# DeepGraphLearning/ultra_torchdrug

Hardware: AMD Instinct MI355X
Metric: edges aggregated/sec, FB15k237-shaped 6L x 64d rspmm Bellman-Ford (predict: the reference's 18 rspmm layers per batch as 6 relation-graph + 6 entity-graph launches, tails and heads in one pass) (higher is better)
Workload: dtype f32

## Files before the change

ultra_torchdrug_amd/csrc/plan_path.h:

```cpp
#ifndef ULTRA_PLAN_PATH_H
#define ULTRA_PLAN_PATH_H

#include <cstddef>
#include <cstdint>

#include "ultra_rspmm.h"

namespace ultra_detail {

constexpr int kTile = 64;
constexpr int kXcd = 8;
constexpr int kMaxLdsBytes = 156 * 1024;
constexpr int kLdsHeader = 16;
constexpr int kPlanBlock = 1024;
constexpr int kPlanRgBlock = 512;

enum Kind { KIND_FWD = 0, KIND_DX = 1, KIND_DREL = 2 };
enum Family { FAM_DENSE = 0, FAM_ROWGROUP = 1, FAM_QUAD = 2, FAM_PACKED = 3, FAM_GENERAL = 4 };
enum RelMode { REL_L2 = 0, REL_LDS = 1, REL_PART = 2 };
enum ActMode { ACT_NONE = 0, ACT_BITS = 2, ACT_NODE = 3 };
enum UnrollClass { UNROLL_U = 0, UNROLL_UW = 1, UNROLL_UX = 2 };
enum Fixup { FIX_NONE = 0, FIX_PLAIN = 1, FIX_MANY = 2 };

struct Knobs {
    bool force_general = false;
    bool no_x_lds = false;
    bool no_quad = false;
    bool no_rowgroup = false;
    bool wide_groups = false;
    bool no_concurrent_tiles = false;
    bool no_dense = false;
    bool no_dead_words = false;
};

inline Knobs decode_knobs(int mask) {
    Knobs k;
    k.force_general = (mask & 1) != 0;
    k.no_x_lds = (mask & 2) != 0;
    k.no_quad = (mask & 4) != 0;
    k.no_rowgroup = (mask & 8) != 0;
    k.wide_groups = (mask & 16) != 0;
    k.no_concurrent_tiles = (mask & 32) != 0;
    k.no_dense = (mask & 64) != 0;
    k.no_dead_words = (mask & 128) != 0;
    return k;
}

inline int gcd_int(int a, int b) {
    while (b) {
        const int t = a % b;
        a = b;
        b = t;
    }
    return a;
}

struct TileGeometry {
    int n_tiles = 0, split = 0, n_slots = 0, blocks_per_label = 0, grid = 0;
};

inline TileGeometry tile_geometry(long long columns, int width, int n_cu) {
    TileGeometry g;
    g.n_tiles = (int)((columns + width - 1) / width);
    g.split = kXcd / gcd_int(g.n_tiles, kXcd);
    g.n_slots = g.n_tiles * g.split;
    g.blocks_per_label = (n_cu + kXcd - 1) / kXcd;
    g.grid = g.blocks_per_label * kXcd;
    return g;
}

struct RowGroupTiling {
    int group = 16;
    int rel_mode = REL_L2;
    int n_rel_lds = 0;
    TileGeometry geo;
    size_t lds = 0;
};

inline RowGroupTiling rowgroup_tiling(long long F, long long gather_rows, long long n_rows, long long n_rel, int n_cu,
                                      bool wide_groups, size_t lds_base, size_t lds_room) {
    RowGroupTiling t;
    const bool dram = wide_groups || (double)gather_rows * (double)F * 4.0 > 256.0 * 1024 * 1024;
    t.group = (dram && F % 256 == 0) ? 64 : ((dram && F % 128 == 0) ? 32 : 16);
    const int width = 4 * t.group;
    t.geo = tile_geometry(F, width, n_cu);
    while ((n_rows + t.geo.split - 1) / t.geo.split * F * 4 >= (1LL << 32) - 65536 && t.geo.split < (1 << 20)) t.geo.split *= 2;
    t.geo.n_slots = t.geo.n_tiles * t.geo.split;
    const size_t row_bytes = (size_t)width * sizeof(float);
    const size_t lds_need = (size_t)n_rel * row_bytes;
    const int part_rows = (int)(lds_room / row_bytes);
    t.lds = lds_base;
    if (n_rel > 0 && lds_need <= lds_room) {
        t.rel_mode = REL_LDS;
        t.n_rel_lds = (int)n_rel;
        t.lds += lds_need;
    } else if (n_rel > 0 && (long long)part_rows * 4 >= n_rel) {
        t.rel_mode = REL_PART;
        t.n_rel_lds = part_rows;
        t.lds += (size_t)part_rows * row_bytes;
    }
    return t;
}

enum Aligned {
    AL_INPUT = 1, AL_GRAD = 2, AL_OUT = 4, AL_RELATION = 8, AL_ADD_ROWS = 16, AL_PARTIAL = 32, AL_BVEC = 64, AL_ALL = 127
};

struct PlanInput {
    int kind = KIND_FWD, sum_op = ULTRA_SUM_ADD, mul_op = ULTRA_MUL_MUL;
    long long F = 0, n_rel = 0, gather_rows = 0, gather2_rows = 0;
    bool has_weight = false, has_node_b = false, has_row_ptr = false, has_packed = false, has_packed_dead = false,
         has_dense = false;
    long long packed_src_shift = 0, n_rows = 0, n_edges = 0, n_long_rows = 0, n_pieces = 0, n_hot = 0, dense_rows = 0,
              dense_cols = 0;
    bool has_add_rows = false, has_bnode = false;
    int bdim = 0;
    bool has_act_bits = false, has_act_node = false;
    int act_words = 0;
    bool has_workspace = false;
    size_t workspace_bytes = 0;
    unsigned aligned = AL_ALL;
    Knobs knobs;
    int n_cu = 0;
    bool gfx950 = false;
};

struct PlanPath {
    int status = ULTRA_OK;
    int family = FAM_GENERAL;
    bool unit_w = false;
    int var = 0;
    bool x_lds = false, dead = false;
    int act = ACT_NONE;
    int unroll = UNROLL_U;
    int concurrent = 1;
    bool rel_lds = false;
    int group = 0, rel_mode = REL_L2, n_rel_lds = 0;
    TileGeometry geo;
    int grid = 0, block = 0;
    size_t lds = 0;
    int fixup = FIX_NONE, fixup_grid = 0;
};

inline void set_rowgroup(PlanPath &r, const RowGroupTiling &t) {
    r.family = FAM_ROWGROUP;
    r.group = t.group; r.rel_mode = t.rel_mode; r.n_rel_lds = t.n_rel_lds;
    r.geo = t.geo; r.grid = t.geo.grid; r.block = kPlanRgBlock; r.lds = t.lds;
}

inline bool dense_applies(const PlanInput &c) {
    if (!c.has_dense || c.has_weight || c.sum_op != ULTRA_SUM_ADD || c.n_rel != 4) return false;
    if (c.F % 16 != 0 || c.F * 4 >= (1LL << 24)) return false;
    if (c.dense_cols != c.gather_rows || c.gather_rows * c.F * 4 >= (1LL << 31)) return false;
    if (c.kind == KIND_DREL) {
        if (c.mul_op != ULTRA_MUL_MUL || c.n_rows != 4 || c.dense_rows != c.gather2_rows) return false;
        const long long n_vt = (c.dense_rows + 15) / 16;
        if (!c.has_workspace || c.workspace_bytes < (size_t)(n_vt * 4 * c.F) * sizeof(float)) return false;
    } else {
        if (c.dense_rows != c.n_rows) return false;
        if (c.kind == KIND_FWD && !c.has_add_rows && c.has_bnode && c.bdim <= 0) return false;
    }
    return true;
}

inline void force_concurrent(PlanPath &path, int want, bool has_min_rows, long long min_rows, long long gather_rows) {
    if (path.family == FAM_QUAD && want >= 1 && path.geo.blocks_per_label % want == 0 && (!has_min_rows || gather_rows >= min_rows))
        path.concurrent = want;
}

inline PlanPath plan_path(const PlanInput &in) {
    PlanPath r;
    const int kind = in.kind;
    const long long F = in.F, n_rel = in.n_rel;
    const Knobs &k = in.knobs;
    auto aligned = [&](unsigned bits) { return (in.aligned & bits) == bits; };
    const unsigned al_gather = (kind == KIND_DX) ? AL_GRAD : AL_INPUT;
    const bool sum_add = in.sum_op == ULTRA_SUM_ADD, mul_mul = in.mul_op == ULTRA_MUL_MUL;
    const bool boundary_ok = !in.has_bnode || in.bdim % 4 == 0;

    r.geo = tile_geometry(F, kTile, in.n_cu);
    r.grid = r.geo.grid;
    r.block = kPlanBlock;
    r.unit_w = !in.has_weight;
    const size_t lds_need = (size_t)n_rel * kTile * sizeof(float);
    const bool rel_fits = n_rel > 0 && lds_need <= (size_t)kMaxLdsBytes;

    if (in.has_dense && !k.no_dense && !k.force_general && !k.no_quad && !k.no_x_lds && in.gfx950 && dense_applies(in)) {
        r.family = FAM_DENSE;
        return r;
    }

    const bool big = in.packed_src_shift >= 32;
    if (kind != KIND_DREL && !k.force_general && !k.no_rowgroup && in.has_row_ptr && big && in.n_long_rows == 0 && F % 4 == 0 &&
        (kind == KIND_FWD || sum_add) && aligned(al_gather | AL_OUT | AL_RELATION | AL_ADD_ROWS | AL_BVEC) && boundary_ok) {
        r.family = FAM_ROWGROUP;
        if (F >= (1LL << 30)) { r.status = ULTRA_ERR_BAD_SHAPE; return r; }
        const bool needs_rel = kind == KIND_FWD || mul_mul;
// ... 81 lines not shown
```

ultra_torchdrug_amd/csrc/rspmm_kernels.hip:

```cpp
#include <hip/hip_runtime.h>
#include <type_traits>

#include <algorithm>
#include <cstdint>
#include <cstdlib>
#include <cstring>
#include <mutex>

#include "host_common.h"
#include "launch_record.h"

thread_local int ultra_detail_last_hip_error = 0;

namespace {

using namespace ultra_detail;

#ifndef ULTRA_BLOCK
#define ULTRA_BLOCK 1024
#endif
constexpr int kBlock = ULTRA_BLOCK;
#ifndef ULTRA_UNROLL
#define ULTRA_UNROLL 8
#endif
// ... 648 lines not shown
        }
#pragma unroll
        for (int q = 0; q < 8; ++q) {
            const int r = 4 * q + (lane >> 4), c = (lane & 15) * 4;
            long long gr = t * kCbRows + r;
            gr = gr < last ? gr : last;
            if constexpr (BND == 0) {
                pa[q] = *reinterpret_cast<const f32x4 *>(p.input + gr * 64 + c);
            } else {
                const unsigned qq = (unsigned)(query0 + r);
                const unsigned step = p.rpn >= kCbRows ? (qq >= (unsigned)p.rpn ? 1u : 0u) : qq / (unsigned)p.rpn;
                const int query = (int)(qq - step * (unsigned)p.rpn);
                const f32x4 zero = {0.0f, 0.0f, 0.0f, 0.0f};
                if constexpr (BND == 1) {
                    const f32x4 v = *reinterpret_cast<const f32x4 *>(bv_lds + query * 64 + c);
                    pa[q] = (node0 + step == (long long)bn_lds[query]) ? v : zero;
                } else {
                    pa[q] = (node0 + step == (long long)p.in_bnode[query]) ? *reinterpret_cast<const f32x4 *>(p.in_bvec + query * 64 + c) : zero;
                }
            }
            pb[q] = *reinterpret_cast<const f32x4 *>(p.update + gr * 64 + c);
        }
    };
    if constexpr (PF) {
        if (wave_global < n_tiles) fetch(wave_global);
    }
    for (long long t = wave_global; t < n_tiles; t += wave_total) {
        const long long row0 = t * kCbRows;
        if constexpr (!PF) fetch(t);
#pragma unroll
        for (int q = 0; q < 8; ++q) {
            const int r = 4 * q + (lane >> 4), c = (lane & 15) * 4;
            *reinterpret_cast<f32x4 *>(tile + r * kCbStride + c) = pa[q];
            *reinterpret_cast<f32x4 *>(tile + r * kCbStride + 64 + c) = pb[q];
        }
        if constexpr (PF) {
            asm volatile("s_waitcnt lgkmcnt(0)" ::: "memory");
            if (t + wave_total < n_tiles) fetch(t + wave_total);
        } else {
            asm volatile("s_waitcnt vmcnt(0) lgkmcnt(0)" ::: "memory");
        }

        f32x16 acc0, acc1;
#pragma unroll
        for (int r = 0; r < 16; ++r) { acc0[r] = bias0; acc1[r] = bias1; }
#pragma unroll
        for (int q = 0; q < 16; ++q) {
            const f32x4 av = *reinterpret_cast<const f32x4 *>(tile + i * kCbStride + 64 * h + 4 * q);
            acc0 = __builtin_amdgcn_mfma_f32_32x32x2f32(av.x, w0[4 * q + 0], acc0, 0, 0, 0);
            acc1 = __builtin_amdgcn_mfma_f32_32x32x2f32(av.x, w1[4 * q + 0], acc1, 0, 0, 0);
            acc0 = __builtin_amdgcn_mfma_f32_32x32x2f32(av.y, w0[4 * q + 1], acc0, 0, 0, 0);
            acc1 = __builtin_amdgcn_mfma_f32_32x32x2f32(av.y, w1[4 * q + 1], acc1, 0, 0, 0);
            acc0 = __builtin_amdgcn_mfma_f32_32x32x2f32(av.z, w0[4 * q + 2], acc0, 0, 0, 0);
            acc1 = __builtin_amdgcn_mfma_f32_32x32x2f32(av.z, w1[4 * q + 2], acc1, 0, 0, 0);
            acc0 = __builtin_amdgcn_mfma_f32_32x32x2f32(av.w, w0[4 * q + 3], acc0, 0, 0, 0);
            acc1 = __builtin_amdgcn_mfma_f32_32x32x2f32(av.w, w1[4 * q + 3], acc1, 0, 0, 0);
        }
        asm volatile("s_waitcnt lgkmcnt(0)" ::: "memory");

#pragma unroll
        for (int r = 0; r < 16; ++r) {
            const int row = (r & 3) + 8 * (r >> 2) + 4 * h;
            tile[row * kCbStride + 64 + i] = acc0[r];
            tile[row * kCbStride + 96 + i] = acc1[r];
        }
        asm volatile("s_waitcnt lgkmcnt(0)" ::: "memory");

        float v[32];
#pragma unroll
        for (int q = 0; q < 8; ++q) {
            const f32x4 d = *reinterpret_cast<const f32x4 *>(tile + ln_row * kCbStride + 64 + 32 * ln_half + 4 * q);
            v[4 * q + 0] = d.x; v[4 * q + 1] = d.y; v[4 * q + 2] = d.z; v[4 * q + 3] = d.w;
            if constexpr (ZOUT) {
                const long long left_z = p.rows - row0;
                const __amdgpu_buffer_rsrc_t rsrc_z = __builtin_amdgcn_make_buffer_rsrc(
                    p.z_out + row0 * 64, 0, (int)(left_z < kCbRows ? left_z : kCbRows) * 256, 0x00020000);
                __builtin_amdgcn_raw_buffer_store_b128(__builtin_bit_cast(qu4, d), rsrc_z, ln_row * 256 + ln_half * 128 + 16 * q, 0, 0);
            }
        }
        if (p.gamma != nullptr) {
            float s = 0.0f;
#pragma unroll
            for (int c = 0; c < 32; ++c) s = s + v[c];
            const float so = __shfl_xor(s, 1, 64);
            const float mean = (ln_half == 0 ? s + so : so + s) * (1.0f / 64.0f);
            float ss = 0.0f;
#pragma unroll
            for (int c = 0; c < 32; ++c) { const float dlt = v[c] - mean; ss = ss + dlt * dlt; }
            const float sso = __shfl_xor(ss, 1, 64);
            const float var = (ln_half == 0 ? ss + sso : sso + ss) * (1.0f / 64.0f);
            const float inv = 1.0f / sqrtf(var + p.eps);
#pragma unroll
            for (int q = 0; q < 8; ++q) {
                const f32x4 gq = *reinterpret_cast<const f32x4 *>(gb + 32 * ln_half + 4 * q);
                const f32x4 bq = *reinterpret_cast<const f32x4 *>(gb + 64 + 32 * ln_half + 4 * q);
                v[4 * q + 0] = ((v[4 * q + 0] - mean) * inv) * gq.x + bq.x;
                v[4 * q + 1] = ((v[4 * q + 1] - mean) * inv) * gq.y + bq.y;
                v[4 * q + 2] = ((v[4 * q + 2] - mean) * inv) * gq.z + bq.z;
                v[4 * q + 3] = ((v[4 * q + 3] - mean) * inv) * gq.w + bq.w;
            }
        }
        if (p.relu) {
#pragma unroll
            for (int c = 0; c < 32; ++c) v[c] = !(v[c] <= 0.0f) ? v[c] : 0.0f;
        }
        if (p.shortcut) {
#pragma unroll
            for (int q = 0; q < 8; ++q) {
                const f32x4 x = *reinterpret_cast<const f32x4 *>(tile + ln_row * kCbStride + 32 * ln_half + 4 * q);
                v[4 * q + 0] = v[4 * q + 0] + x.x; v[4 * q + 1] = v[4 * q + 1] + x.y;
                v[4 * q + 2] = v[4 * q + 2] + x.z; v[4 * q + 3] = v[4 * q + 3] + x.w;
            }
        }
#pragma unroll
        for (int q = 0; q < 8; ++q) {
            f32x4 d;
            d.x = v[4 * q + 0]; d.y = v[4 * q + 1]; d.z = v[4 * q + 2]; d.w = v[4 * q + 3];
            *reinterpret_cast<f32x4 *>(tile + ln_row * kCbStride + 64 + 32 * ln_half + 4 * q) = d;
        }
        asm volatile("s_waitcnt lgkmcnt(0)" ::: "memory");

        if constexpr (BND == 3) {
            if (p.rows * 256 >= (1LL << 32) - 65536) {
#pragma unroll
                for (int q = 0; q < 8; ++q) {
                    const int r = 4 * q + (lane >> 4), c = (lane & 15) * 4;
                    const f32x4 d = *reinterpret_cast<const f32x4 *>(tile + r * kCbStride + 64 + c);
                    if (rid[q] >= 0) *reinterpret_cast<f32x4 *>(p.out + (long long)rid[q] * 64 + c) = d;
                }
                asm volatile("s_waitcnt lgkmcnt(0)" ::: "memory");
                continue;
            }
            const __amdgpu_buffer_rsrc_t rsrc_all = __builtin_amdgcn_make_buffer_rsrc(p.out, 0, (int)(uint32_t)(p.rows * 256), 0x00020000);
#pragma unroll
            for (int q = 0; q < 8; ++q) {
                const int r = 4 * q + (lane >> 4), c = (lane & 15) * 4;
                const f32x4 d = *reinterpret_cast<const f32x4 *>(tile + r * kCbStride + 64 + c);
                const uint32_t off = rid[q] >= 0 ? (uint32_t)rid[q] * 256u + (uint32_t)c * 4u : 0xffffffffu;
                __builtin_amdgcn_raw_buffer_store_b128(__builtin_bit_cast(qu4, d), rsrc_all, off, 0, 0);
            }
            asm volatile("s_waitcnt lgkmcnt(0)" ::: "memory");
            continue;
        }
        const long long left = p.rows - row0;
        const __amdgpu_buffer_rsrc_t rsrc_tile = __builtin_amdgcn_make_buffer_rsrc(
            p.out + row0 * 64, 0, (int)(left < kCbRows ? left : kCbRows) * 256, 0x00020000);
#pragma unroll
        for (int q = 0; q < 8; ++q) {
            const int r = 4 * q + (lane >> 4), c = (lane & 15) * 4;
            const f32x4 d = *reinterpret_cast<const f32x4 *>(tile + r * kCbStride + 64 + c);
            __builtin_amdgcn_raw_buffer_store_b128(__builtin_bit_cast(qu4, d), rsrc_tile, r * 256 + c * 4, 0, 0);
        }
        asm volatile("s_waitcnt lgkmcnt(0)" ::: "memory");
    }
}


static_assert(kBlock == kPlanBlock && kRgBlock == kPlanRgBlock, "plan_path.h states the workgroup sizes of its families");
static_assert(kRelL2 == REL_L2 && kRelLds == REL_LDS && kRelPart == REL_PART, "plan_path.h's RelMode is rowgroup.inc's REL");

thread_local hipEvent_t g_prof_start = nullptr;
thread_local hipEvent_t g_prof_stop = nullptr;
#ifndef ULTRA_QUAD_U
#define ULTRA_QUAD_U 8
#endif
constexpr int kQuadU = ULTRA_QUAD_U;
#ifndef ULTRA_QUAD_UW
#define ULTRA_QUAD_UW 6
#endif
constexpr int kQuadUW = ULTRA_QUAD_UW;
#ifndef ULTRA_QUAD_UX
#define ULTRA_QUAD_UX 8
#endif
constexpr int kQuadUX = ULTRA_QUAD_UX;

thread_local LaunchRing g_launches;

template <typename Kern, typename Params>
int launch_recorded(LaunchRecord rec, Kern kern, const Params &p, int grid, size_t lds, hipStream_t stream, int block) {
    rec.grid = grid; rec.block = block; rec.lds = (int32_t)lds;
    rec.n_tiles = p.n_tiles; rec.split = p.split; rec.n_slots = p.n_slots; rec.blocks_per_label = p.blocks_per_label;
    LaunchRecord &slot = g_launches.push(rec);
    return slot.status = launch_with_lds(kern, p, grid, lds, stream, block);
}


template <int KIND, int SUM, int MUL>
int launch_general(const KParams &p, const PlanPath &path, hipStream_t stream) {
    return with_bool(path.unit_w, [&](auto uw) {
        return with_bool(path.rel_lds, [&](auto rl) {
            constexpr bool UW = decltype(uw)::value, RL = decltype(rl)::value;
            if constexpr (RL && (KIND == KIND_DREL || (KIND == KIND_DX && SUM == ULTRA_SUM_ADD && MUL == ULTRA_MUL_ADD)))
                return (int)ULTRA_ERR_BAD_OP;
            else {
                LaunchRecord rec;
                rec.family = FAM_GENERAL; rec.kind = KIND; rec.sum = SUM; rec.mul = MUL; rec.unit_w = UW; rec.rel_lds = RL;
                return launch_recorded(rec, segment_kernel<KIND, SUM, MUL, UW, RL>, p, path.grid, path.lds, stream, kBlock);
            }
        });
    });
}

template <int KIND, int SUM, int MUL>
int launch_packed(const PParams &p, const PlanPath &path, hipStream_t stream) {
    return with_bool(path.unit_w, [&](auto uw) {
        auto go = [&](auto var) {
            constexpr int V = decltype(var)::value;
            constexpr int UN = (V == 2 || V == 3) ? kUnrollBig : kUnroll;
            constexpr bool UW = decltype(uw)::value;
            if constexpr (KIND == KIND_DX && MUL == ULTRA_MUL_ADD && V == 2) return (int)ULTRA_ERR_BAD_OP;
            else {
                LaunchRecord rec;
                rec.family = FAM_PACKED; rec.kind = KIND; rec.sum = SUM; rec.mul = MUL; rec.unit_w = UW; rec.var = V; rec.unroll = UN;
                return launch_recorded(rec, packed_kernel<KIND, SUM, MUL, UW, V, UN>, p, path.grid, path.lds, stream, kBlock);
            }
        };
        if constexpr (KIND == KIND_DREL) return go(std::integral_constant<int, 0>{});
        else return with_int<0, 1, 2, 3, 4>(path.var, go);
    });
}

template <int KIND, int SUM, int MUL>
int launch_quad(const PParams &p, const PlanPath &path, hipStream_t stream) {
#define ULTRA_Q(UW, XL, U, ACT, DEAD)                                                                                          \
    do {                                                                                                                       \
        LaunchRecord rec;                                                                                                      \
        rec.family = FAM_QUAD; rec.kind = KIND; rec.sum = SUM; rec.mul = MUL; rec.unit_w = UW; rec.x_lds = XL; rec.unroll = U; \
        rec.act = ACT; rec.dead = DEAD; rec.concurrent = p.concurrent;                                                         \
        return launch_recorded(rec, quad_kernel<KIND, SUM, MUL, UW, XL, U, ACT, DEAD>, p, path.grid, path.lds, stream, kBlock); \
    } while (0)
    if constexpr (SUM == ULTRA_SUM_ADD && MUL == ULTRA_MUL_MUL) {
        if (path.dead) {
            if constexpr (KIND == KIND_DREL) {
                if (path.act == ACT_BITS) ULTRA_Q(true, false, kQuadU, 2, true);
            }
            ULTRA_Q(true, false, kQuadU, 0, true);
        }
    }
    if constexpr (KIND == KIND_DREL) {
        if (path.act == ACT_BITS) {
            if (path.unit_w) ULTRA_Q(true, false, kQuadU, 2, false);
            ULTRA_Q(false, false, kQuadUW, 2, false);
        }
        if constexpr (MUL == ULTRA_MUL_MUL) {
            if (path.act == ACT_NODE) {
                if (path.unit_w) ULTRA_Q(true, false, kQuadU, 3, false);
                ULTRA_Q(false, false, kQuadUW, 3, false);
            }
        }
    }
    if constexpr (KIND != KIND_DREL || MUL == ULTRA_MUL_MUL) {
        if (path.x_lds) {
            if (path.unit_w) ULTRA_Q(true, true, kQuadUX, 0, false);
            ULTRA_Q(false, true, kQuadUW, 0, false);
        }
    }
    if (path.unit_w) ULTRA_Q(true, false, kQuadU, 0, false);
    ULTRA_Q(false, false, kQuadUW, 0, false);
#undef ULTRA_Q
}

template <int SUM, int MUL, bool BACKWARD>
int launch_rowgroup(const RowGroupParams &p, const PlanPath &path, hipStream_t stream) {
    constexpr bool NEEDS_REL = !BACKWARD || MUL == ULTRA_MUL_MUL;
    return with_int<16, 32, 64>(path.group, [&](auto g) {
        return with_bool(path.unit_w, [&](auto uw) {
            return with_int<kRelL2, kRelLds, kRelPart>(path.rel_mode, [&](auto rel) {
                constexpr int REL = decltype(rel)::value;
                if constexpr (!NEEDS_REL && REL != kRelL2) return (int)ULTRA_ERR_BAD_OP;
                else {
                    constexpr bool UW = decltype(uw)::value;
                    constexpr int G = decltype(g)::value;
                    LaunchRecord rec;
                    rec.family = FAM_ROWGROUP; rec.kind = BACKWARD ? KIND_DX : KIND_FWD; rec.sum = SUM; rec.mul = MUL; rec.unit_w = UW;
                    rec.rel_mode = REL; rec.group = G; rec.needs_rel = NEEDS_REL; rec.backward = BACKWARD; rec.n_rel_lds = p.n_rel_lds;
                    return launch_recorded(rec, rowgroup_kernel<SUM, MUL, UW, REL, NEEDS_REL, BACKWARD, G>, p, path.grid, path.lds, stream,
                                           kRgBlock);
                }
            });
        });
    });
}

void fill_tiling(RowGroupParams &q, const PlanPath &path) {
    q.n_tiles = path.geo.n_tiles;
    q.split = path.geo.split;
    q.n_slots = path.geo.n_slots;
    q.blocks_per_label = path.geo.blocks_per_label;
    q.n_rel_lds = path.n_rel_lds;
}

template <int KIND, typename Fn>
int with_fast_ops(int sum_op, int mul_op, Fn &&fn) {
    if constexpr (KIND == KIND_FWD) return with_sum_mul(sum_op, mul_op, fn);
    else return with_mul(mul_op, [&](auto mul) { return fn(std::integral_constant<int, ULTRA_SUM_ADD>{}, mul); });
}

inline bool aligned16(const void *ptr) { return (reinterpret_cast<uintptr_t>(ptr) & 15u) == 0; }

template <int KIND>
int launch_words(const ultra_segments *seg, const KParams &p, const PlanPath &path, int64_t gather_rows, int64_t gather2_rows,
                 int64_t n_rel, int64_t F, int sum_op, int mul_op, hipStream_t stream) {
    const bool big = seg->packed_src_shift >= 32;
    const bool quad = path.family == FAM_QUAD;
    const unsigned long long relation_bytes = (unsigned long long)n_rel * (unsigned long long)F * 4ull;
    const unsigned long long meta_bytes = ((unsigned long long)seg->n_edges + 16ull) * 4ull;
// ... 646 lines not shown
        int rc = run_plan<KIND_DREL>(by_rel, p, n_src, n_dst, n_rel, F, sum_op, mul_op, workspace, workspace_bytes, s);
        if (rc) return rc;
    }
    return ULTRA_OK;
}

int ultra_rspmm_backward_f32(const ultra_segments *by_src, const ultra_segments *by_rel, const float *relation,
                             const float *input, const float *output, const float *output_grad, float *d_input,
                             float *d_relation, void *workspace, size_t workspace_bytes, int64_t n_src, int64_t n_dst,
                             int64_t n_rel, int64_t F, int sum_op, int mul_op, void *stream) {
    return ultra_rspmm_backward_accumulate_f32(by_src, by_rel, relation, input, output, output_grad, nullptr, d_input,
                                               d_relation, workspace, workspace_bytes, n_src, n_dst, n_rel, F, sum_op,
                                               mul_op, stream);
}

int ultra_rspmm_backward_accumulate_f32(const ultra_segments *by_src, const ultra_segments *by_rel, const float *relation,
                                        const float *input, const float *output, const float *output_grad,
                                        const float *d_input_add, float *d_input, float *d_relation, void *workspace,
                                        size_t workspace_bytes, int64_t n_src, int64_t n_dst, int64_t n_rel, int64_t F,
                                        int sum_op, int mul_op, void *stream) {
    if (output_grad == nullptr || relation == nullptr || input == nullptr) return ULTRA_ERR_NULL_POINTER;
    if (d_input_add != nullptr && sum_op != ULTRA_SUM_ADD) return ULTRA_ERR_BAD_OP;
    if (sum_op != ULTRA_SUM_ADD && output == nullptr) return ULTRA_ERR_NULL_POINTER;
    return backward_plans(by_src, by_rel, relation, input, output, output_grad, d_input_add, d_input, d_relation, workspace,
                          workspace_bytes, n_src, n_dst, n_rel, F, sum_op, mul_op, nullptr, 0, nullptr, static_cast<hipStream_t>(stream));
}

int ultra_rspmm_backward_active_f32(const ultra_segments *by_src, const ultra_segments *by_rel, const float *relation,
                                    const float *input, const float *output_grad, const float *d_input_add, float *d_input,
                                    float *d_relation, void *workspace, size_t workspace_bytes, int64_t n_src, int64_t n_dst,
                                    int64_t n_rel, int64_t F, int mul_op, const uint32_t *dst_active_bits, int64_t active_words,
                                    const int32_t *src_active_node, void *stream) {
    if (output_grad == nullptr || relation == nullptr || input == nullptr) return ULTRA_ERR_NULL_POINTER;
    if (dst_active_bits != nullptr && (active_words < (n_dst + 31) / 32 || active_words > 0x7fffffffLL)) return ULTRA_ERR_BAD_SHAPE;
    if ((dst_active_bits != nullptr || src_active_node != nullptr) && F % kTile != 0) return ULTRA_ERR_BAD_SHAPE;
    return backward_plans(by_src, by_rel, relation, input, nullptr, output_grad, d_input_add, d_input, d_relation, workspace,
                          workspace_bytes, n_src, n_dst, n_rel, F, ULTRA_SUM_ADD, mul_op, dst_active_bits, active_words,
                          src_active_node, static_cast<hipStream_t>(stream));
}

int ultra_rspmm_backward_weight_f32(const ultra_segments *fwd, const float *relation, const float *input,
                                    const float *output, const float *output_grad, float *d_weight, int64_t n_rel,
                                    int64_t F, int sum_op, int mul_op, void *stream) {
    int rc = check_segments(fwd);
    if (rc) return rc;
    (void)n_rel;
    if (F <= 0) return ULTRA_ERR_BAD_SHAPE;
    if (sum_op < 0 || sum_op > 2 || mul_op < 0 || mul_op > 1) return ULTRA_ERR_BAD_OP;
    if (fwd->n_edges == 0) return ULTRA_OK;
    if (relation == nullptr || input == nullptr || output_grad == nullptr || d_weight == nullptr)
        return ULTRA_ERR_NULL_POINTER;
    if (sum_op != ULTRA_SUM_ADD && output == nullptr) return ULTRA_ERR_NULL_POINTER;
    hipStream_t s = static_cast<hipStream_t>(stream);
    const bool unit = fwd->weight == nullptr;
    long long blocks = (fwd->n_edges + 3) / 4;
    if (blocks > 8192) blocks = 8192;
    return with_sum_mul(sum_op, mul_op, [&](auto sum, auto mul) {
        return with_bool(unit, [&](auto uw) -> int {
            hipLaunchKernelGGL((weight_grad_kernel<decltype(sum)::value, decltype(mul)::value, decltype(uw)::value>), dim3((int)blocks),
                               dim3(256), 0, s, fwd->row, fwd->node_a, fwd->rel, fwd->weight, relation, input, output, output_grad,
                               d_weight, (long long)F, (long long)fwd->n_edges);
            HIP_TRY(hipGetLastError());
            return ULTRA_OK;
        });
    });
}

int ultra_rspmm_rotate_forward_f32(const ultra_segments *fwd, const float *relation, const float *input,
                                   const float *add_rows, const int32_t *boundary_node, const float *boundary_value,
                                   float *out, void *workspace, size_t workspace_bytes, int64_t n_src, int64_t n_rel,
                                   int64_t F, int64_t block, int sum_op, void *stream) {
    (void)n_src;
    if (fwd == nullptr) return ULTRA_ERR_NULL_POINTER;
    if (!segments_abi_ok(fwd)) return ULTRA_ERR_ABI;
    if (fwd->n_rows > 0 && out == nullptr) return ULTRA_ERR_NULL_POINTER;
    if (fwd->n_edges > 0 && (relation == nullptr || input == nullptr)) return ULTRA_ERR_NULL_POINTER;
    if ((boundary_node == nullptr) != (boundary_value == nullptr)) return ULTRA_ERR_NULL_POINTER;
    if (boundary_node != nullptr && add_rows != nullptr) return ULTRA_ERR_BAD_SHAPE;
    RotParams p{};
    p.relation = relation;
    p.input = input;
    p.add_rows = add_rows;
    p.bnode = boundary_node;
    p.bvec = boundary_value;
    p.out = out;
    return run_rotate_plan<KIND_FWD>(fwd, p, n_rel, F, block, sum_op, workspace, workspace_bytes,
                                     static_cast<hipStream_t>(stream));
}

int ultra_rspmm_rotate_backward_f32(const ultra_segments *by_src, const ultra_segments *by_rel, const float *relation,
                                    const float *input, const float *output, const float *output_grad, float *d_input,
                                    float *d_relation, void *workspace, size_t workspace_bytes, int64_t n_src,
                                    int64_t n_dst, int64_t n_rel, int64_t F, int64_t block, int sum_op, void *stream) {
    (void)n_src;
    (void)n_dst;
    if (by_src != nullptr && !segments_abi_ok(by_src)) return ULTRA_ERR_ABI;
    if (by_rel != nullptr && !segments_abi_ok(by_rel)) return ULTRA_ERR_ABI;
    if (block <= 0 || block % 2 != 0 || F <= 0 || F % block != 0) return ULTRA_ERR_BAD_SHAPE;
    if (sum_op < 0 || sum_op > 2) return ULTRA_ERR_BAD_OP;
    if (output_grad == nullptr || relation == nullptr || input == nullptr) return ULTRA_ERR_NULL_POINTER;
    if (sum_op != ULTRA_SUM_ADD && output == nullptr) return ULTRA_ERR_NULL_POINTER;
    hipStream_t s = static_cast<hipStream_t>(stream);
    if (d_input != nullptr) {
        if (by_src == nullptr) return ULTRA_ERR_NULL_POINTER;
        RotParams p{};
        p.relation = relation; p.input = input; p.output = output; p.grad = output_grad; p.out = d_input;
        int rc = run_rotate_plan<KIND_DX>(by_src, p, n_rel, F, block, sum_op, workspace, workspace_bytes, s);
        if (rc) return rc;
    }
    if (d_relation != nullptr) {
        if (by_rel == nullptr) return ULTRA_ERR_NULL_POINTER;
        if (by_rel->n_edges > 0 && by_rel->node_b == nullptr) return ULTRA_ERR_NULL_POINTER;
        RotParams p{};
        p.relation = relation; p.input = input; p.output = output; p.grad = output_grad; p.out = d_relation;
        int rc = run_rotate_plan<KIND_DREL>(by_rel, p, n_rel, F, block, sum_op, workspace, workspace_bytes, s);
        if (rc) return rc;
    }
    return ULTRA_OK;
}

int ultra_rspmm_rotate_backward_weight_f32(const ultra_segments *fwd, const float *relation, const float *input,
                                           const float *output, const float *output_grad, float *d_weight, int64_t n_rel,
                                           int64_t F, int64_t block, int sum_op, void *stream) {
    int rc = check_segments(fwd);
    if (rc) return rc;
    (void)n_rel;
    if (F <= 0 || F > 0x7ffffffeLL || block <= 0 || block % 2 != 0 || F % block != 0) return ULTRA_ERR_BAD_SHAPE;
    if (sum_op < 0 || sum_op > 2) return ULTRA_ERR_BAD_OP;
    if (fwd->n_edges == 0) return ULTRA_OK;
    if (relation == nullptr || input == nullptr || output_grad == nullptr || d_weight == nullptr)
        return ULTRA_ERR_NULL_POINTER;
    if (sum_op != ULTRA_SUM_ADD && output == nullptr) return ULTRA_ERR_NULL_POINTER;
    hipStream_t s = static_cast<hipStream_t>(stream);
    const int half = (int)(block / 2);
    return with_sum(sum_op, [&](auto sum) {
        return launch_rotate_weight_grad<decltype(sum)::value>(fwd, relation, input, output, output_grad, d_weight, F, half, s);
    });
}


static int combine_launch(const CombineParams &p, void *stream) {
    DeviceInfo *di = nullptr;
    int rc = current_device_info(&di);
    if (rc) return rc;
    const long long n_tiles = (p.rows + kCbRows - 1) / kCbRows;
    long long blocks = (n_tiles + kCbWaves - 1) / kCbWaves;
    const bool prefetch = n_tiles >= (long long)di->n_cu * kCbWaves * 4;
    const long long resident = (long long)di->n_cu * (prefetch ? 1 : 2);
    if (blocks > resident) blocks = resident;
    const bool bnd_lds = p.in_bnode != nullptr && p.rpn <= kCbLdsQueries;
    const int lds_max = (int)((kCbWaves * kCbTileFloats + 128 + kCbLdsQueries * 65) * sizeof(float));
    const size_t lds = (size_t)(kCbWaves * kCbTileFloats + 128 + (bnd_lds ? p.rpn * 65 : 0)) * sizeof(float);
    hipStream_t st = static_cast<hipStream_t>(stream);
    return with_bool(prefetch, [&](auto pf) {
        constexpr bool PF = decltype(pf)::value;
        auto go = [&](auto kern) { return launch_with_lds(kern, p, (int)blocks, lds, st, kCbWaves * 64, lds_max); };
        if (bnd_lds) return go(combine_kernel<PF, 1>);
        if (p.in_bnode != nullptr) return go(combine_kernel<PF, 2>);
        if (p.z_out != nullptr) return go(combine_kernel<PF, 0, true>);
        return go(combine_kernel<PF, 0>);
    });
}

int ultra_combine_forward_f32(const float *input, const float *update, const float *weight, const float *bias,
                              const float *ln_weight, const float *ln_bias, float ln_eps, int relu, int shortcut,
                              float *out, float *z_out, int64_t rows, int64_t dim, void *stream) {
    if (dim != 64) return ULTRA_ERR_BAD_SHAPE;
    if (rows < 0) return ULTRA_ERR_BAD_SHAPE;
    if (rows == 0) return ULTRA_OK;
    if (input == nullptr || update == nullptr || weight == nullptr || bias == nullptr || out == nullptr)
        return ULTRA_ERR_NULL_POINTER;
    if (ln_weight != nullptr && ln_bias == nullptr) return ULTRA_ERR_NULL_POINTER;
    CombineParams p{};
    p.input = input; p.update = update; p.weight = weight; p.bias = bias; p.gamma = ln_weight; p.beta = ln_bias;
    p.out = out; p.rows = rows; p.eps = ln_eps; p.relu = relu; p.shortcut = shortcut;
    p.z_out = z_out;
    return combine_launch(p, stream);
}

int ultra_combine_forward_boundary_f32(const int32_t *boundary_node, const float *boundary_value, int64_t n_query,
                                       const float *update, const float *weight, const float *bias, const float *ln_weight,
                                       const float *ln_bias, float ln_eps, int relu, int shortcut, float *out, int64_t rows,
                                       int64_t dim, void *stream) {
    if (dim != 64 || rows < 0 || n_query <= 0 || n_query > 0x7fffffffLL || rows % n_query != 0) return ULTRA_ERR_BAD_SHAPE;
    if (rows == 0) return ULTRA_OK;
    if (boundary_node == nullptr || boundary_value == nullptr || update == nullptr || weight == nullptr || bias == nullptr ||
        out == nullptr)
        return ULTRA_ERR_NULL_POINTER;
    if (ln_weight != nullptr && ln_bias == nullptr) return ULTRA_ERR_NULL_POINTER;
    if (reinterpret_cast<uintptr_t>(boundary_value) & 15u) return ULTRA_ERR_BAD_SHAPE;
    CombineParams p{};
    p.input = nullptr; p.update = update; p.weight = weight; p.bias = bias; p.gamma = ln_weight; p.beta = ln_bias;
    p.out = out; p.rows = rows; p.eps = ln_eps; p.relu = relu; p.shortcut = shortcut;
    p.in_bnode = boundary_node; p.in_bvec = boundary_value; p.rpn = (int)n_query;
    return combine_launch(p, stream);
}

}

#include "combine_train.inc"
#include "combine_fused_bwd.inc"
#include "first_layer_train.inc"
#include "dense.inc"
#include "project_bwd.inc"
#include "sampler.inc"
#include "guard.inc"
#include "score_rows.inc"
```

Before: 44.31 billion.

## Add paired-wave combine kernel with register/LDS-split weight and dynamic tile tickets

Adds a combine kernel that keeps half of the 64x64 linear weight in registers and the other half in LDS. Each wave computes two 32-column output halves with f32 MFMA. Tiles are handed out through a workgroup-local atomic ticket, and the next tile is prefetched while the current one is processed. It runs for large row counts when no boundary-node or z_out outputs are requested. The aim is to cut weight reloads and improve latency hiding in the combine (linear + layernorm + relu + shortcut) step, at the cost of heavy register pressure at one workgroup per CU.

Result: faster. 45.04 billion, median of 6 (+1.6%).

```diff
diff --git a/ultra_torchdrug_amd/csrc/plan_path.h b/ultra_torchdrug_amd/csrc/plan_path.h
--- a/ultra_torchdrug_amd/csrc/plan_path.h
+++ b/ultra_torchdrug_amd/csrc/plan_path.h
@@ -31,6 +31,8 @@
     bool no_concurrent_tiles = false;
     bool no_dense = false;
     bool no_dead_words = false;
+    bool no_paired = false;
+    bool force_paired = false;
 };
 
 inline Knobs decode_knobs(int mask) {
@@ -43,6 +45,8 @@
     k.no_concurrent_tiles = (mask & 32) != 0;
     k.no_dense = (mask & 64) != 0;
     k.no_dead_words = (mask & 128) != 0;
+    k.no_paired = (mask & 256) != 0;
+    k.force_paired = (mask & 512) != 0;
     return k;
 }
 
diff --git a/ultra_torchdrug_amd/csrc/rspmm_kernels.hip b/ultra_torchdrug_amd/csrc/rspmm_kernels.hip
--- a/ultra_torchdrug_amd/csrc/rspmm_kernels.hip
+++ b/ultra_torchdrug_amd/csrc/rspmm_kernels.hip
@@ -824,6 +824,177 @@
             __builtin_amdgcn_raw_buffer_store_b128(__builtin_bit_cast(qu4, d), rsrc_tile, r * 256 + c * 4, 0, 0);
         }
         asm volatile("s_waitcnt lgkmcnt(0)" ::: "memory");
+    }
+}
+
+constexpr int kCpWaves = 8;
+constexpr int kCpW1Floats = 32 * kCbStride;
+constexpr int kCpLdsFloats = kCpWaves * kCbTileFloats + kCpW1Floats + 128 + 4;
+constexpr int kCpMinTilesPerGroup = 16;
+static_assert(kCpLdsFloats * sizeof(float) <= (size_t)kMaxLdsBytes, "eight tiles and half the weight fit one CU's LDS");
+
+__global__ __launch_bounds__(kCpWaves * 64, 1) void combine_paired_kernel(const CombineParams p) {
+    extern __shared__ __attribute__((aligned(16))) float cb_lds[];
+    const int lane = threadIdx.x & 63;
+    const int wl = uniform(threadIdx.x >> 6);
+    float *tile = cb_lds + wl * kCbTileFloats;
+    float *w1_lds = cb_lds + kCpWaves * kCbTileFloats;
+    float *gb = w1_lds + kCpW1Floats;
+    int *ticket = reinterpret_cast<int *>(gb + 128);
+    const int i = lane & 31, h = lane >> 5;
+    const long long n_tiles = (p.rows + kCbRows - 1) / kCbRows;
+    const long long lo = n_tiles * blockIdx.x / gridDim.x;
+    const int n_mine = (int)(n_tiles * (blockIdx.x + 1) / gridDim.x - lo);
+
+    float w0[64];
+#pragma unroll
+    for (int q = 0; q < 16; ++q) {
+        const f32x4 a = *reinterpret_cast<const f32x4 *>(p.weight + (long long)i * 128 + 64 * h + 4 * q);
+        w0[4 * q + 0] = a.x; w0[4 * q + 1] = a.y; w0[4 * q + 2] = a.z; w0[4 * q + 3] = a.w;
+    }
+    for (int j = threadIdx.x; j < 32 * 32; j += kCpWaves * 64)
+        *reinterpret_cast<f32x4 *>(w1_lds + (j >> 5) * kCbStride + 4 * (j & 31)) =
+            *reinterpret_cast<const f32x4 *>(p.weight + (long long)(32 + (j >> 5)) * 128 + 4 * (j & 31));
+    const float bias0 = p.bias[i], bias1 = p.bias[i + 32];
+    const int ln_row = lane >> 1, ln_half = lane & 1;
+    if (p.gamma != nullptr && threadIdx.x < 128) gb[threadIdx.x] = threadIdx.x < 64 ? p.gamma[threadIdx.x] : p.beta[threadIdx.x - 64];
+    if (threadIdx.x == 0) *ticket = 0;
+    __syncthreads();
+
+    const long long last = p.rows - 1;
+    f32x4 pa[8], pb[8];
+    auto fetch = [&](long long t) {
+#pragma unroll
+        for (int q = 0; q < 8; ++q) {
+            const int r = 4 * q + (lane >> 4), c = (lane & 15) * 4;
+            long long gr = t * kCbRows + r;
+            gr = gr < last ? gr : last;
+            pa[q] = *reinterpret_cast<const f32x4 *>(p.input + gr * 64 + c);
+            pb[q] = *reinterpret_cast<const f32x4 *>(p.update + gr * 64 + c);
+        }
+    };
+    auto draw = [&]() {
+        int t = 0;
+        if (lane == 0) t = __hip_atomic_fetch_add(ticket, 1, __ATOMIC_RELAXED, __HIP_MEMORY_SCOPE_WORKGROUP);
+        return t;
+    };
+    int cur = uniform(draw());
+    if (cur >= n_mine) return;
+    fetch(lo + cur);
+    {
+        const __amdgpu_buffer_rsrc_t rsrc_none = __builtin_amdgcn_make_buffer_rsrc(p.out, 0, 0, 0x00020000);
+        const f32x4 zero = {0.0f, 0.0f, 0.0f, 0.0f};
+#pragma unroll
+        for (int q = 0; q < 8; ++q)
+            __builtin_amdgcn_raw_buffer_store_b128(__builtin_bit_cast(qu4, zero), rsrc_none, (4 * q + (lane >> 4)) * 256 + (lane & 15) * 16, 0, 0);
+    }
+    while (cur < n_mine) {
+        const long long row0 = (lo + cur) * kCbRows;
+        const int drawn = draw();
+#pragma unroll
+        for (int q = 0; q < 8; ++q) {
+            const int r = 4 * q + (lane >> 4), c = (lane & 15) * 4;
+            *reinterpret_cast<f32x4 *>(tile + r * kCbStride + c) = pa[q];
+            *reinterpret_cast<f32x4 *>(tile + r * kCbStride + 64 + c) = pb[q];
+        }
+        asm volatile("s_waitcnt lgkmcnt(0)" ::: "memory");
+        const int nxt = uniform(drawn);
+        fetch(nxt < n_mine ? lo + nxt : n_tiles);
+
+        float b0 = bias0, b1 = bias1;
+        asm volatile("" : "+v"(b0), "+v"(b1));
+        f32x16 acc0, acc1;
+#pragma unroll
+        for (int r = 0; r < 16; ++r) { acc0[r] = b0; acc1[r] = b1; }
+        f32x4 av = *reinterpret_cast<const f32x4 *>(tile + i * kCbStride + 64 * h);
+        f32x4 bv = *reinterpret_cast<const f32x4 *>(w1_lds + i * kCbStride + 64 * h);
+#pragma unroll
+        for (int q = 0; q < 16; ++q) {
+            f32x4 an = av, bn = bv;
+            if (q < 15) {
+                an = *reinterpret_cast<const f32x4 *>(tile + i * kCbStride + 64 * h + 4 * (q + 1));
+                bn = *reinterpret_cast<const f32x4 *>(w1_lds + i * kCbStride + 64 * h + 4 * (q + 1));
+            }
+            acc0 = __builtin_amdgcn_mfma_f32_32x32x2f32(av.x, w0[4 * q + 0], acc0, 0, 0, 0);
+            acc1 = __builtin_amdgcn_mfma_f32_32x32x2f32(av.x, bv.x, acc1, 0, 0, 0);
+            acc0 = __builtin_amdgcn_mfma_f32_32x32x2f32(av.y, w0[4 * q + 1], acc0, 0, 0, 0);
+            acc1 = __builtin_amdgcn_mfma_f32_32x32x2f32(av.y, bv.y, acc1, 0, 0, 0);
+            acc0 = __builtin_amdgcn_mfma_f32_32x32x2f32(av.z, w0[4 * q + 2], acc0, 0, 0, 0);
+            acc1 = __builtin_amdgcn_mfma_f32_32x32x2f32(av.z, bv.z, acc1, 0, 0, 0);
+            acc0 = __builtin_amdgcn_mfma_f32_32x32x2f32(av.w, w0[4 * q + 3], acc0, 0, 0, 0);
+            acc1 = __builtin_amdgcn_mfma_f32_32x32x2f32(av.w, bv.w, acc1, 0, 0, 0);
+            __builtin_amdgcn_sched_barrier(0);
+            av = an; bv = bn;
+        }
+        asm volatile("s_waitcnt lgkmcnt(0)" ::: "memory");
+
+#pragma unroll
+        for (int r = 0; r < 16; ++r) {
+            const int row = (r & 3) + 8 * (r >> 2) + 4 * h;
+            tile[row * kCbStride + 64 + i] = acc0[r];
+            tile[row * kCbStride + 96 + i] = acc1[r];
+        }
+        asm volatile("s_waitcnt lgkmcnt(0)" ::: "memory");
+
+        float v[32];
+#pragma unroll
+        for (int q = 0; q < 8; ++q) {
+            const f32x4 d = *reinterpret_cast<const f32x4 *>(tile + ln_row * kCbStride + 64 + 32 * ln_half + 4 * q);
+            v[4 * q + 0] = d.x; v[4 * q + 1] = d.y; v[4 * q + 2] = d.z; v[4 * q + 3] = d.w;
+        }
+        if (p.gamma != nullptr) {
+            float s = 0.0f;
+#pragma unroll
+            for (int c = 0; c < 32; ++c) s = s + v[c];
+            const float so = __shfl_xor(s, 1, 64);
+            const float mean = (ln_half == 0 ? s + so : so + s) * (1.0f / 64.0f);
+            float ss = 0.0f;
+#pragma unroll
+            for (int c = 0; c < 32; ++c) { const float dlt = v[c] - mean; ss = ss + dlt * dlt; }
+            const float sso = __shfl_xor(ss, 1, 64);
+            const float var = (ln_half == 0 ? ss + sso : sso + ss) * (1.0f / 64.0f);
+            const float inv = 1.0f / sqrtf(var + p.eps);
+#pragma unroll
+            for (int q = 0; q < 8; ++q) {
+                const f32x4 gq = *reinterpret_cast<const f32x4 *>(gb + 32 * ln_half + 4 * q);
+                const f32x4 bq = *reinterpret_cast<const f32x4 *>(gb + 64 + 32 * ln_half + 4 * q);
+                v[4 * q + 0] = ((v[4 * q + 0] - mean) * inv) * gq.x + bq.x;
+                v[4 * q + 1] = ((v[4 * q + 1] - mean) * inv) * gq.y + bq.y;
+                v[4 * q + 2] = ((v[4 * q + 2] - mean) * inv) * gq.z + bq.z;
+                v[4 * q + 3] = ((v[4 * q + 3] - mean) * inv) * gq.w + bq.w;
+            }
+        }
+        if (p.relu) {
+#pragma unroll
+            for (int c = 0; c < 32; ++c) v[c] = !(v[c] <= 0.0f) ? v[c] : 0.0f;
+        }
+        if (p.shortcut) {
+#pragma unroll
+            for (int q = 0; q < 8; ++q) {
+                const f32x4 x = *reinterpret_cast<const f32x4 *>(tile + ln_row * kCbStride + 32 * ln_half + 4 * q);
+                v[4 * q + 0] = v[4 * q + 0] + x.x; v[4 * q + 1] = v[4 * q + 1] + x.y;
+                v[4 * q + 2] = v[4 * q + 2] + x.z; v[4 * q + 3] = v[4 * q + 3] + x.w;
+            }
+        }
+#pragma unroll
+        for (int q = 0; q < 8; ++q) {
+            f32x4 d;
+            d.x = v[4 * q + 0]; d.y = v[4 * q + 1]; d.z = v[4 * q + 2]; d.w = v[4 * q + 3];
+            *reinterpret_cast<f32x4 *>(tile + ln_row * kCbStride + 64 + 32 * ln_half + 4 * q) = d;
+        }
+        asm volatile("s_waitcnt lgkmcnt(0)" ::: "memory");
+
+        const long long left = p.rows - row0;
+        const __amdgpu_buffer_rsrc_t rsrc_tile = __builtin_amdgcn_make_buffer_rsrc(
+            p.out + row0 * 64, 0, (int)(left < kCbRows ? left : kCbRows) * 256, 0x00020000);
+#pragma unroll
+        for (int q = 0; q < 8; ++q) {
+            const int r = 4 * q + (lane >> 4), c = (lane & 15) * 4;
+            const f32x4 d = *reinterpret_cast<const f32x4 *>(tile + r * kCbStride + 64 + c);
+            __builtin_amdgcn_raw_buffer_store_b128(__builtin_bit_cast(qu4, d), rsrc_tile, r * 256 + c * 4, 0, 0);
+        }
+        asm volatile("s_waitcnt lgkmcnt(0)" ::: "memory");
+        cur = nxt;
     }
 }
 
@@ -1776,6 +1947,12 @@
     const int lds_max = (int)((kCbWaves * kCbTileFloats + 128 + kCbLdsQueries * 65) * sizeof(float));
     const size_t lds = (size_t)(kCbWaves * kCbTileFloats + 128 + (bnd_lds ? p.rpn * 65 : 0)) * sizeof(float);
     hipStream_t st = static_cast<hipStream_t>(stream);
+    if (p.in_bnode == nullptr && p.z_out == nullptr && !g_knobs.no_paired && (prefetch || g_knobs.force_paired)) {
+        long long groups = n_tiles / kCpMinTilesPerGroup;
+        groups = groups < 1 ? 1 : (groups > di->n_cu ? di->n_cu : groups);
+        if (n_tiles / groups < 0x7fffff00LL)
+            return launch_with_lds(combine_paired_kernel, p, (int)groups, kCpLdsFloats * sizeof(float), st, kCpWaves * 64);
+    }
     return with_bool(prefetch, [&](auto pf) {
         constexpr bool PF = decltype(pf)::value;
         auto go = [&](auto kern) { return launch_with_lds(kern, p, (int)blocks, lds, st, kCbWaves * 64, lds_max); };
```
